# deezer/musicFPaugment

Measured on AMD Instinct MI355X. Metric: 8s/8kHz clips/sec (STFT+UNet+peak-pick), higher is better.
Workload: dtype bf16x3 (fp32 operands split into bf16 hi+lo, fp32 accumulate); 1 GPU; STFT(512/256,f64) -> UNet(1,1) eval forward (bf16x3 MFMA, formula weights) -> Audfprint peak-pick; 8 s / 8 kHz clips, 257x251 spectrograms; parallelism=clip-sharded x1, no data-path collective

## Files before the change

musicfpaugment_amd/csrc/unet.hip:

```cpp
#include "mfpa_common.h"
#include "mfpa_unet_args.h"

#include <cstdlib>
#include <type_traits>

namespace {

#ifdef MFPA_EXPERIMENTS
__device__ unsigned long long* mfpa_conv_stamps = nullptr;
#define MFPA_STAMP(slot)                                                                                                   \
  do {                                                                                                                     \
    if (mfpa_conv_stamps && threadIdx.x == 0)                                                                              \
      mfpa_conv_stamps[((size_t)blockIdx.y * gridDim.x + blockIdx.x) * 8 + (slot)] = __builtin_amdgcn_s_memrealtime();   \
  } while (0)
#else
#define MFPA_STAMP(slot) do { } while (0)
#endif

typedef float floatx16 __attribute__((ext_vector_type(16)));
typedef float f32x4 __attribute__((ext_vector_type(4)));
typedef __bf16 bf16x8 __attribute__((ext_vector_type(8)));
typedef __bf16 bf16x4 __attribute__((ext_vector_type(4)));
typedef __bf16 bf16x2 __attribute__((ext_vector_type(2)));
typedef float f32x2 __attribute__((ext_vector_type(2)));
// ... 591 lines not shown
    }
  }
  MFPA_STAMP(4);
}

typedef float floatx4 __attribute__((ext_vector_type(4)));

template <int CTRL>
__device__ __forceinline__ float dpp_row_add(float v) {
  return v + __int_as_float(__builtin_amdgcn_update_dpp(0, __float_as_int(v), CTRL, 0xf, 0xf, false));
}

template <int PH, int PW, bool ROWS, int WMW = 2, bool SIDE = false, bool PLAIN = false, bool IN16 = false, bool AFF16 = false>
__global__ __launch_bounds__(512, 1) void conv_wd16_kernel(ConvArgs a) {
  static_assert(!IN16 || PLAIN, "a bf16 source feeds the plain-bf16 products");
  constexpr int SPP = IN16 ? KC / 8 : KC / 4;
  constexpr int ESZ = IN16 ? 2 : 4;
  constexpr int THREADS = 512, WNW = 8 / WMW, BN = 32 * WNW, WPXW = 256 / WMW, TAPS = 9;
  static_assert((WMW == 2 || WMW == 4) && (!ROWS || WMW == 2), "wave grid");
  constexpr int HPW = PW + 2, HPH = PH + 2, HP = HPW * HPH, BM = PH * PW;
  static_assert(BM == 256 && (PW == 32 || PW == 16), "two waves of 128 pixels: eight 16-pixel tiles each");
  constexpr int A_F4 = (HP * SPP + THREADS - 1) / THREADS;
  constexpr int HPS = A_F4 * (THREADS / SPP);
  constexpr int PLANE = ((HPS * 16 + 255) / 256) * 256;
  constexpr int HLS = 4 * PLANE + 256;
  constexpr int STAGE = 2 * HLS;
  constexpr int PT = WPXW / 16;
  static_assert(A_F4 <= TAPS - 3, "one halo staging slot per tap, taps 2 .. 7");

  extern __shared__ __attribute__((aligned(16))) char smem[];
  const int tid = threadIdx.x, lane = tid & 63, wave = tid >> 6;
  const int wm = wave % WMW, wn = __builtin_amdgcn_readfirstlane(wave / WMW);
  const int p = lane & 15, g = lane >> 4;
  auto plane_off = [](int hl, int kg) { return hl * HLS + kg * PLANE + (kg >> 1) * 128; };

  constexpr bool PERSIST = (WMW == 4) || (!ROWS && !SIDE) || PLAIN;
  const int n0 = blockIdx.y * BN;
  const int Cin = a.C0 + a.C1;
  const int nchunks = Cin / KC;
  const int ntiles = a.tiles_x * a.tiles_y * a.B;

  const int aq = tid % SPP;
  constexpr int TBL = 2 * A_F4 * THREADS;
  unsigned* const aoffs0 = reinterpret_cast<unsigned*>(smem + 2 * STAGE);
#pragma unroll
  for (int it = 0; it < A_F4; ++it) {
    const int pix = tid / SPP + it * (THREADS / SPP);
    const int py = pix / HPW - 1, px = pix % HPW - 1;
    aoffs0[it * THREADS + tid] = (unsigned)((py * a.W + px) * a.C0 + (KC / SPP) * aq) * (unsigned)ESZ;
    aoffs0[(A_F4 + it) * THREADS + tid] = (unsigned)(((py - a.oy1) * a.W1 + (px - a.ox1)) * a.C1 + (KC / SPP) * aq) * (unsigned)ESZ;
  }
  typedef int i32x4_t __attribute__((ext_vector_type(4)));
  const unsigned clip0 = (unsigned)a.H * (unsigned)a.W * (unsigned)a.C0 * (unsigned)ESZ, clip1 = (unsigned)a.H1 * (unsigned)a.W1 * (unsigned)a.C1 * (unsigned)ESZ;
  struct Tile { int b, y0, x0p; unsigned ain; unsigned t0, t1; };
  auto make_tile = [&](int t) __attribute__((always_inline)) {
    Tile T;
    int bx = __builtin_amdgcn_readfirstlane(t);
// ... 101 lines not shown
        const float* scp = aff + c0 + 8 * aq;
        const float* shp = aff + a.C0 + c0 + 8 * aq;
        const f32x4 sc0 = *reinterpret_cast<const f32x4*>(scp), sc1 = *reinterpret_cast<const f32x4*>(scp + 4);
        const f32x4 sh0 = *reinterpret_cast<const f32x4*>(shp), sh1 = *reinterpret_cast<const f32x4*>(shp + 4);
#pragma unroll
        for (int k = 0; k < 8; ++k) {
          const float y = f[k] * (k < 4 ? sc0[k & 3] : sc1[k & 3]) + (k < 4 ? sh0[k & 3] : sh1[k & 3]);
          f[k] = y > 0.f ? y : 0.f;
        }
        if (a.drop_thresh) {
          const int gy = S.y0 + pix / HPW - 1, gx = S.x0p + pix % HPW - 1;
          const unsigned long long e0 = (((unsigned long long)S.b * a.H + gy) * a.W + gx) * a.C0 + c0 + 8 * aq;
#pragma unroll
          for (int k = 0; k < 8; ++k) f[k] = mfpa_keep(a.drop_seed, a.drop_thresh, e0 + k) ? f[k] * a.drop_scale : 0.f;
        }
#pragma unroll
        for (int k = 0; k < 4; ++k) {
          bf16x2 h2;
          h2[0] = (__bf16)f[2 * k];
          h2[1] = (__bf16)f[2 * k + 1];
          v[k] = __builtin_bit_cast(float, h2);
        }
      }
      *reinterpret_cast<f32x4*>(stage + plane_off(0, aq) + pix * 16) = v;
      if constexpr (SIDE && AFF16) {
        const int py = pix / HPW, px = pix % HPW;
        if (a.x0_bf16 != nullptr && c0 < a.C0 && inside && py >= 1 && py <= PH && px >= 1 && px <= PW && blockIdx.y == 0) {
          const size_t e = (size_t)S.b * a.H * a.W * a.C0 + ((aoffs0[it * THREADS + tid] + S.t0) >> 1) + c0;
          *reinterpret_cast<f32x4*>(a.x0_bf16 + e) = v;
        }
      }
      return;
    }
    if (a.in_scale0 != nullptr && c0 < a.C0 && inside) {
      const f32x4 sc = *reinterpret_cast<const f32x4*>(aff + c0 + 4 * aq);
      const f32x4 sh = *reinterpret_cast<const f32x4*>(aff + a.C0 + c0 + 4 * aq);
      v = v * sc + sh;
#pragma unroll
      for (int k = 0; k < 4; ++k) v[k] = v[k] > 0.f ? v[k] : 0.f;
      if (a.drop_thresh) {
        const int gy = S.y0 + pix / HPW - 1, gx = S.x0p + pix % HPW - 1;
        const unsigned long long e0 = (((unsigned long long)S.b * a.H + gy) * a.W + gx) * a.C0 + c0 + 4 * aq;
#pragma unroll
        for (int k = 0; k < 4; ++k) v[k] = mfpa_keep(a.drop_seed, a.drop_thresh, e0 + k) ? v[k] * a.drop_scale : 0.f;
      }
    }
    bf16x4 hi, lo;
#pragma unroll
    for (int k = 0; k < 4; ++k) {
      hi[k] = (__bf16)v[k];
      lo[k] = (__bf16)(v[k] - (float)hi[k]);
    }
    char* at = stage + plane_off(0, aq >> 1) + pix * 16 + 8 * (aq & 1);
    *reinterpret_cast<bf16x4*>(at) = hi;
    if constexpr (!PLAIN) *reinterpret_cast<bf16x4*>(at + HLS) = lo;
    if constexpr (SIDE) {
      const int py = pix / HPW, px = pix % HPW;
      const bool interior = inside && py >= 1 && py <= PH && px >= 1 && px <= PW && blockIdx.y == 0;
      if (a.x0_bf16 != nullptr && c0 < a.C0 && interior) {
        const size_t e = (size_t)S.b * a.H * a.W * a.C0 + ((aoffs0[it * THREADS + tid] + S.t0) >> 2) + c0;
        *reinterpret_cast<bf16x4*>(a.x0_bf16 + e) = hi;
      }
      if (a.x1_bf16 != nullptr && c0 >= a.C0 && interior) {
        const size_t e = (size_t)S.b * a.H1 * a.W1 * a.C1 + ((aoffs0[(A_F4 + it) * THREADS + tid] + S.t1) >> 2) + (c0 - a.C0);
        *reinterpret_cast<bf16x4*>(a.x1_bf16 + e) = hi;
      }
    }
  };

  bf16x8 wq[3][2][2];
  auto load_w = [&](int chunk, int tap, auto SLOT) __attribute__((always_inline)) {
    constexpr int slot = decltype(SLOT)::value;
    const char* wb = reinterpret_cast<const char*>(a.w) +
                     ((((size_t)tap * nchunks + chunk) * (size_t)(a.Cout / 16) + (size_t)(n0 / 16 + 2 * wn)) << 11) + lane * 16;
    wq[slot][0][0] = *reinterpret_cast<const bf16x8*>(wb);
    if constexpr (!PLAIN) wq[slot][0][1] = *reinterpret_cast<const bf16x8*>(wb + 1024);
    wq[slot][1][0] = *reinterpret_cast<const bf16x8*>(wb + 2048);
    if constexpr (!PLAIN) wq[slot][1][1] = *reinterpret_cast<const bf16x8*>(wb + 3072);
  };

  struct XFrags { bf16x8 h[4], l[4]; };
  XFrags fx0, fx1;
  const int xbase = (((wm * WPXW + p) / PW) * HPW + ((wm * WPXW + p) % PW)) * 16 + plane_off(0, g);
  auto tile_disp = [](int pt) { return (PW == 32) ? ((pt >> 1) * HPW + (pt & 1) * 16) * 16 : pt * HPW * 16; };
  auto read_x = [&](XFrags& f, const char* stage, int tap_off, int half) __attribute__((always_inline)) {
#pragma unroll
    for (int i = 0; i < 4; ++i) {
      const char* r = stage + xbase + tile_disp(4 * half + i) + tap_off;
      if constexpr (!PLAIN) f.l[i] = *reinterpret_cast<const bf16x8*>(r + HLS);
      f.h[i] = *reinterpret_cast<const bf16x8*>(r);
    }
  };
  floatx4 acc[2][PT];
#pragma unroll
  for (int ct = 0; ct < 2; ++ct)
#pragma unroll
    for (int pt = 0; pt < PT; ++pt) acc[ct][pt] = floatx4{0.f, 0.f, 0.f, 0.f};
  auto mfma_half = [&](const XFrags& f, const bf16x8 (&w)[2][2], int half) __attribute__((always_inline)) {
    if constexpr (!PLAIN) {
#pragma unroll
    for (int ct = 0; ct < 2; ++ct)
#pragma unroll
      for (int i = 0; i < 4; ++i) acc[ct][4 * half + i] = __builtin_amdgcn_mfma_f32_16x16x32_bf16(w[ct][1], f.h[i], acc[ct][4 * half + i], 0, 0, 0);
#pragma unroll
    for (int ct = 0; ct < 2; ++ct)
#pragma unroll
      for (int i = 0; i < 4; ++i) acc[ct][4 * half + i] = __builtin_amdgcn_mfma_f32_16x16x32_bf16(w[ct][0], f.l[i], acc[ct][4 * half + i], 0, 0, 0);
    }
#pragma unroll
    for (int ct = 0; ct < 2; ++ct)
#pragma unroll
      for (int i = 0; i < 4; ++i) acc[ct][4 * half + i] = __builtin_amdgcn_mfma_f32_16x16x32_bf16(w[ct][0], f.h[i], acc[ct][4 * half + i], 0, 0, 0);
  };
  using S0 = std::integral_constant<int, 0>;
  using S1 = std::integral_constant<int, 1>;
  constexpr int N_R = PLAIN ? 4 : 8, N_M = PLAIN ? 8 : 24;
  constexpr int N_W = PLAIN ? 2 : 4;
  auto tap_body = [&](auto TAP, int chunk) __attribute__((always_inline)) {
    constexpr int tap = decltype(TAP)::value;
    constexpr int ntap = (tap + 1) % TAPS;
    constexpr int tap_off = ((tap / 3) * HPW + (tap % 3)) * 16, ntap_off = ((ntap / 3) * HPW + (ntap % 3)) * 16;
    const int chunk_n = chunk + 1 < nchunks ? chunk + 1 : (PERSIST ? 0 : chunk);
    const char* cur = smem + (chunk & 1) * STAGE;
    const char* nxt = (tap == TAPS - 1) ? smem + ((chunk + 1) & 1) * STAGE : cur;
    read_x(fx1, cur, tap_off, 1);
    mfma_half(fx0, wq[tap % 3], 0);
    load_w((tap + 2 >= TAPS) ? chunk_n : chunk, (tap + 2) % TAPS, std::integral_constant<int, (tap + 2) % 3>{});
    pin_reads<N_M - 1, N_R>();
    constexpr int used_a = pin_read_slots(N_M - 1, N_R);
    __builtin_amdgcn_sched_group_barrier(0x008, 1, 0);
    __builtin_amdgcn_sched_group_barrier(0x020, N_W, 0);
    if constexpr (N_M - used_a - 1 > 0) __builtin_amdgcn_sched_group_barrier(0x008, N_M - used_a - 1, 0);
    __builtin_amdgcn_sched_barrier(0);
    if (tap == TAPS - 1) {
      __syncthreads();
      __builtin_amdgcn_sched_barrier(0);
    }
    if (tap == 0) load_a_pre(chunk_n);
    if (tap == TAPS - 1) preload_offsets(PERSIST ? (chunk + 2 < nchunks ? chunk + 2 : chunk + 1 < nchunks ? 0 : 1 < nchunks ? 1 : 0)
                                                 : (chunk + 2 < nchunks ? chunk + 2 : chunk + 1 < nchunks ? chunk + 1 : chunk));
    read_x(fx0, nxt, ntap_off, 0);
    mfma_half(fx1, wq[tap % 3], 1);
    if constexpr (tap >= 2 && tap - 2 < A_F4) {
      split_slot(std::integral_constant<int, tap - 2>{}, chunk_n, smem + ((chunk + 1) & 1) * STAGE);
#pragma unroll
      for (int i = 0; i < N_R; ++i) {
        __builtin_amdgcn_sched_group_barrier(0x008, 1, 0);
        __builtin_amdgcn_sched_group_barrier(0x100, 1, 0);
        __builtin_amdgcn_sched_group_barrier(0x002, 2, 0);
      }
#pragma unroll
      for (int i = 0; i < 2; ++i) {
        __builtin_amdgcn_sched_group_barrier(0x008, 2, 0);
        __builtin_amdgcn_sched_group_barrier(0x002, 4, 0);
        __builtin_amdgcn_sched_group_barrier(0x200, 1, 0);
      }
      if constexpr (N_M - N_R - 4 > 0) __builtin_amdgcn_sched_group_barrier(0x008, N_M - N_R - 4, 0);
    } else {
      pin_reads<N_M, N_R>();
      if constexpr (N_M - pin_read_slots(N_M, N_R) > 0) __builtin_amdgcn_sched_group_barrier(0x008, N_M - pin_read_slots(N_M, N_R), 0);
    }
    __builtin_amdgcn_sched_barrier(0);
  };

  auto tap_body4 = [&](auto TAP, auto PAR, int chunk) __attribute__((always_inline)) {
    constexpr int tap = decltype(TAP)::value, par = (decltype(PAR)::value + tap) & 1;
    constexpr int ntap = (tap + 1) % TAPS;
    constexpr int ntap_off = ((ntap / 3) * HPW + (ntap % 3)) * 16;
    const int chunk_n = chunk + 1 < nchunks ? chunk + 1 : 0;
    const char* cur = smem + (chunk & 1) * STAGE;
    const char* nxt = (tap == TAPS - 1) ? smem + ((chunk + 1) & 1) * STAGE : cur;
    stamp(tap);
    if (tap == TAPS - 1) {
      __syncthreads();
      __builtin_amdgcn_sched_barrier(0);
      stamp(9);
    }
    if (tap == 0) load_a_pre(chunk_n);
    if (tap == TAPS - 1) preload_offsets(chunk + 2 < nchunks ? chunk + 2 : chunk + 1 < nchunks ? 0 : 1 < nchunks ? 1 : 0);
    read_x(par ? fx0 : fx1, nxt, ntap_off, 0);
    if (!MFPA_EXP_FLAG(a.dbg, 8)) mfma_half(par ? fx1 : fx0, wq[tap % 3], 0);
    if (!MFPA_EXP_FLAG(a.dbg, 128)) load_w((tap + 2 >= TAPS) ? chunk_n : chunk, (tap + 2) % TAPS, std::integral_constant<int, (tap + 2) % 3>{});
    if constexpr (tap >= 2 && tap - 2 < A_F4) {
      if (!MFPA_EXP_FLAG(a.dbg, 256)) split_slot(std::integral_constant<int, tap - 2>{}, chunk_n, smem + ((chunk + 1) & 1) * STAGE);
#pragma unroll
      for (int i = 0; i < N_R; ++i) {
        __builtin_amdgcn_sched_group_barrier(0x008, 1, 0);
        __builtin_amdgcn_sched_group_barrier(0x100, 1, 0);
        __builtin_amdgcn_sched_group_barrier(0x002, 2, 0);
      }
#pragma unroll
// ... 33 lines not shown
    for (int dy = 0; dy < 3; ++dy) {
      const char* wb = reinterpret_cast<const char*>(a.w) +
                       ((((size_t)(dy * 3 + dx) * nchunks + chunk) * (size_t)(a.Cout / 16) + (size_t)(n0 / 16 + 2 * wn)) << 11) + lane * 16;
      wr[par][dy][0][0] = *reinterpret_cast<const bf16x8*>(wb);
      if constexpr (!PLAIN) wr[par][dy][0][1] = *reinterpret_cast<const bf16x8*>(wb + 1024);
      wr[par][dy][1][0] = *reinterpret_cast<const bf16x8*>(wb + 2048);
      if constexpr (!PLAIN) wr[par][dy][1][1] = *reinterpret_cast<const bf16x8*>(wb + 3072);
    }
  };
  constexpr int NU = (R + 2) * HV, NB = (PW == 32) ? 4 : 5;
  static_assert(NU % NB == 0, "static ring indices");
  auto load_wr1 = [&](int chunk, auto DX, auto PAR, auto DY) __attribute__((always_inline)) {
    constexpr int dx = decltype(DX)::value, par = decltype(PAR)::value, dy = decltype(DY)::value;
    const char* wb = reinterpret_cast<const char*>(a.w) +
                     ((((size_t)(dy * 3 + dx) * nchunks + chunk) * (size_t)(a.Cout / 16) + (size_t)(n0 / 16 + 2 * wn)) << 11) + lane * 16;
    wr[par][dy][0][0] = *reinterpret_cast<const bf16x8*>(wb);
    if constexpr (!PLAIN) wr[par][dy][0][1] = *reinterpret_cast<const bf16x8*>(wb + 1024);
    wr[par][dy][1][0] = *reinterpret_cast<const bf16x8*>(wb + 2048);
    if constexpr (!PLAIN) wr[par][dy][1][1] = *reinterpret_cast<const bf16x8*>(wb + 3072);
  };
  struct XUnit { bf16x8 h, l; };
  XUnit xu[NB];
  auto read_unit = [&](XUnit& f, const char* stage, int u, int dx) __attribute__((always_inline)) {
    const char* r = stage + xbase + ((u / HV) * HPW + (u % HV) * 16 + dx) * 16;
    if constexpr (!PLAIN) f.l = *reinterpret_cast<const bf16x8*>(r + HLS);
    f.h = *reinterpret_cast<const bf16x8*>(r);
  };
  auto mfma_unit = [&](auto U, const XUnit& f, auto PAR) __attribute__((always_inline)) {
    constexpr int h = decltype(U)::value / HV, hv = decltype(U)::value % HV, par = decltype(PAR)::value;
#pragma unroll
    for (int term = PLAIN ? 2 : 0; term < 3; ++term)
#pragma unroll
      for (int dy = 0; dy < 3; ++dy) {
        if (h - dy < 0 || h - dy >= R) continue;
#pragma unroll
        for (int ct = 0; ct < 2; ++ct) {
          floatx4& c = acc[ct][(h - dy) * HV + hv];
          c = __builtin_amdgcn_mfma_f32_16x16x32_bf16(wr[par][dy][ct][term == 0 ? 1 : 0], term == 1 ? f.l : f.h, c, 0, 0, 0);
        }
      }
  };
  auto unit_mfmas = [](int u) { const int h = u / HV; int n = 0; for (int dy = 0; dy < 3; ++dy) n += (h - dy >= 0 && h - dy < R) ? 1 : 0; return n * (PLAIN ? 2 : 6); };
  constexpr int BARU = NU - NB + 1;
  constexpr int SA = NU / 2, SB = BARU - AHALF;
  static_assert(SA + AHALF < NU && SB >= 0, "staging schedule");
  auto unit_step = [&](auto U, auto DX, auto PAR, int chunk) __attribute__((always_inline)) {
    constexpr int u = decltype(U)::value, dx = decltype(DX)::value, par = decltype(PAR)::value;
// ... 375 lines not shown
    tap_body(std::integral_constant<int, 5>{}, chunk);
    tap_body(std::integral_constant<int, 6>{}, chunk);
    tap_body(std::integral_constant<int, 7>{}, chunk);
    tap_body(std::integral_constant<int, 8>{}, chunk);
  }
  epilogue();
  }
}

constexpr int CONV_WD16_ROWS = 512;

template <int PH, int PW, int WMW = 2>
int launch_wd16(ConvArgs& a, hipStream_t s) {
  a.tiles_x = (a.W + PW - 1) / PW;
  a.tiles_y = (a.H + PH - 1) / PH;
  static const int dbg_env = MFPA_EXP_ENV("MFPA_CONV_DBG", 0);
  a.dbg = dbg_env;
  static const int stagger_env = MFPA_EXP_ENV("MFPA_CONV_STAGGER", 0);
  a.dbg_stagger = stagger_env;
  if ((long long)a.tiles_x * a.tiles_y * a.B > 0x7fffffffLL) return MFPA_EINVAL;
  constexpr int HP = (PW + 2) * (PH + 2);
  constexpr int A_F4 = (HP * (KC / 4) + 511) / 512;
  constexpr int HPS = A_F4 * 64;
  constexpr int PLANE = ((HPS * 16 + 255) / 256) * 256;
  const size_t lds = 2 * (size_t)(2 * (4 * PLANE + 256)) + (size_t)2 * A_F4 * 512 * sizeof(unsigned) +
                     (a.in_scale0 ? (size_t)2 * a.C0 * sizeof(float) : 0) +
                     (a.w1x1 ? (size_t)2 * 256 * sizeof(float) : 0) +
                     (size_t)(2 * 32 * (8 / WMW) + 64) * sizeof(float);
  dim3 grid((unsigned)((long long)a.tiles_x * a.tiles_y * a.B), (unsigned)(a.Cout / (32 * (8 / WMW))));
#ifdef MFPA_EXPERIMENTS
  a.dbg_lds_stamps = (int)lds;
  const_cast<size_t&>(lds) += 4096;
#endif
  const int cin = a.C0 + a.C1;
  const bool side = a.x0_bf16 || a.x1_bf16 || a.y_bf16 || a.stats_part;
  const bool rows = WMW == 2 && cin % 64 == 0 && cin >= CONV_WD16_ROWS;
  if (WMW == 4 || a.plain || (!side && !rows)) {
    const int cus = mfpa_current_device_cus();
    const unsigned per = (unsigned)((cus > 0 ? cus : 256) / (int)grid.y);
    if (per >= 1 && grid.x > per) grid.x = per;
  }
  if (a.in16) {
    if (!a.plain || a.x1_bf16 || cin % 64) return MFPA_EINVAL;
    const bool fwd16 = a.in_scale0 != nullptr || a.x0_bf16 != nullptr || (a.y == nullptr && a.bz == nullptr);
    if constexpr (WMW == 4) {
      if (fwd16) hipLaunchKernelGGL((conv_wd16_kernel<PH, PW, false, 4, true, true, true, true>), grid, dim3(512), lds, s, a);
      else if (side) hipLaunchKernelGGL((conv_wd16_kernel<PH, PW, false, 4, true, true, true>), grid, dim3(512), lds, s, a);
      else hipLaunchKernelGGL((conv_wd16_kernel<PH, PW, false, 4, false, true, true>), grid, dim3(512), lds, s, a);
// ... 656 lines not shown
```

musicfpaugment_amd/csrc/unet_up.hip:

```cpp
#include "mfpa_common.h"
#include "mfpa_unet_args.h"

#include <type_traits>

namespace mfpa_unet {
namespace {

typedef float f32x4 __attribute__((ext_vector_type(4)));
typedef float floatx4 __attribute__((ext_vector_type(4)));
typedef __bf16 bf16x8 __attribute__((ext_vector_type(8)));
typedef float f32x2 __attribute__((ext_vector_type(2)));
typedef __bf16 bf16x2 __attribute__((ext_vector_type(2)));

constexpr int KC = 32;
constexpr int PH = 8, PW = 32, HPW = PW + 2, HPH = PH + 2, HP = HPW * HPH;
constexpr int HALF = HPW / 2;
constexpr int LPH = PH / 2 + 2, LPW = PW / 2 + 2, LP = LPH * LPW;
constexpr int THREADS = 512, LTHREADS = 256;
constexpr int SPP = KC / 4;
constexpr int PPI = LTHREADS / SPP;
constexpr int A_F4 = (HP + PPI - 1) / PPI;
constexpr int L_F4 = (LP + PPI - 1) / PPI;
constexpr int HPS = A_F4 * PPI;
constexpr int PLANE = ((HPS * 16 + 255) / 256) * 256;
constexpr int HLS = 4 * PLANE + 256;
constexpr int STAGE = 2 * HLS;
constexpr int PT = 8;
constexpr int EPI_FLOATS = 64 + 16 * 64;
constexpr int OUTBUF = PH * PW * 64 * 4;

__device__ __forceinline__ constexpr int plane_off(int hl, int kg) { return hl * HLS + kg * PLANE + (kg >> 1) * 128; }

template <int SLOTS, int LEFT, int I = 0>
__device__ __forceinline__ void pin_reads() {
  if constexpr (I < SLOTS && LEFT > 0) {
    constexpr int k = (LEFT + (SLOTS - I) - 1) / (SLOTS - I);
    __builtin_amdgcn_sched_group_barrier(0x008, 1, 0);
    __builtin_amdgcn_sched_group_barrier(0x100, k, 0);
    pin_reads<SLOTS, LEFT - k, I + 1>();
  }
}
constexpr int pin_read_slots(int slots, int left) {
  int used = 0;
  for (int i = 0; i < slots && left > 0; ++i) {
    left -= (left + (slots - i) - 1) / (slots - i);
    ++used;
  }
  return used;
}

__device__ __forceinline__ int tile_of(int b, int i, int G, int ngrp) {
  if (ngrp == 1 && (G & 7) == 0) return i * G + (b & 7) * (G >> 3) + (b >> 3);
  return i * G + b;
}
// ... 94 lines not shown
    }
    const unsigned clip0 = (unsigned)a.H * (unsigned)a.W * (unsigned)a.Cs * 4u, clip1 = (unsigned)a.Hl * (unsigned)a.Wl * (unsigned)a.Cl * 4u;
    f32x4 areg[2][A_F4] = {};
    struct Src { __amdgpu_buffer_rsrc_t rs; unsigned toff; bool from0, interior; int ainsh; };
    auto make_src = [&](const Tile& T, int chunk) __attribute__((always_inline)) {
      Src S;
      S.from0 = chunk < nsk;
      const char* pb = reinterpret_cast<const char*>(S.from0 ? a.skip : a.low) + (size_t)T.b * (S.from0 ? clip0 : clip1);
      S.rs = __builtin_amdgcn_make_buffer_rsrc(const_cast<char*>(pb), 0, (int)(S.from0 ? clip0 : clip1), 0x00020000);
      S.toff = S.from0 ? T.t0 + (unsigned)(chunk * KC) * 4u : T.t1 + (unsigned)((chunk - nsk) * KC) * 4u;
      S.interior = S.from0 ? T.int0 : T.int1;
      S.ainsh = S.from0 ? 0 : 16;
      return S;
    };
    auto issue_slot = [&](const Src& S, unsigned ain, unsigned tab, auto INTERIOR, auto SET, auto IT) __attribute__((always_inline)) {
      constexpr int it = decltype(IT)::value, set = decltype(SET)::value;
      if constexpr (decltype(INTERIOR)::value) {
        areg[set][it] = __builtin_bit_cast(f32x4, __builtin_amdgcn_raw_buffer_load_b128(S.rs, (int)tab, (int)S.toff, 0));
      } else {
        const bool inside = (ain >> (S.ainsh + it)) & 1u;
        areg[set][it] = __builtin_bit_cast(f32x4, __builtin_amdgcn_raw_buffer_load_b128(S.rs, (int)(inside ? tab + S.toff : 0xfffffff0u), 0, 0));
      }
    };
    char* const wbase = smem + plane_off(0, aq >> 1) + pl * 16 + 8 * (aq & 1);
    char* const wbase32 = smem + plane_off(aq >> 2, aq & 3) + pl * 16;
    auto split_slot = [&](auto SET, auto IT, int stage_off) __attribute__((always_inline)) {
      constexpr int it = decltype(IT)::value, set = decltype(SET)::value;
      const f32x4 v = areg[set][it];
      if constexpr (PREC == 0) {
        *reinterpret_cast<f32x4*>(wbase32 + stage_off + it * PPI * 16) = v;
        return;
      }
      unsigned hi[2], lo[2];
#pragma unroll
      for (int h = 0; h < 2; ++h) {
        const f32x2 x = {v[2 * h], v[2 * h + 1]};
        hi[h] = __builtin_bit_cast(unsigned, __builtin_convertvector(x, bf16x2));
        const f32x2 r = {x[0] - __uint_as_float(hi[h] << 16), x[1] - __uint_as_float(hi[h] & 0xffff0000u)};
        lo[h] = __builtin_bit_cast(unsigned, __builtin_convertvector(r, bf16x2));
      }
      char* at = wbase + stage_off + it * PPI * 16;
      *reinterpret_cast<uint2*>(at) = uint2{hi[0], hi[1]};
      *reinterpret_cast<uint2*>(at + HLS) = uint2{lo[0], lo[1]};
    };
    static_assert(A_F4 == 11 && L_F4 == 4, "eleven / four staging slots per loader thread");
#define MFPA_UP_EACH4(M) M(0) M(1) M(2) M(3)
#define MFPA_UP_EACH7(M) M(4) M(5) M(6) M(7) M(8) M(9) M(10)
    auto issue_all = [&](const Src& S, unsigned ain, auto SET) __attribute__((always_inline)) {
      if (S.from0) {
        if (S.interior) {
#define MFPA_UP_ISSUE(I) issue_slot(S, ain, off0[I], std::true_type{}, SET, std::integral_constant<int, I>{});
          MFPA_UP_EACH4(MFPA_UP_ISSUE) MFPA_UP_EACH7(MFPA_UP_ISSUE)
#undef MFPA_UP_ISSUE
        } else {
#define MFPA_UP_ISSUE(I) issue_slot(S, ain, off0[I], std::false_type{}, SET, std::integral_constant<int, I>{});
          MFPA_UP_EACH4(MFPA_UP_ISSUE) MFPA_UP_EACH7(MFPA_UP_ISSUE)
#undef MFPA_UP_ISSUE
        }
      } else {
        if (S.interior) {
#define MFPA_UP_ISSUE(I) issue_slot(S, ain, off1[I], std::true_type{}, SET, std::integral_constant<int, I>{});
          MFPA_UP_EACH4(MFPA_UP_ISSUE)
#undef MFPA_UP_ISSUE
        } else {
// ... 52 lines not shown
  const int wlane = lane * 16;
  auto load_w_at = [&](__amdgpu_buffer_rsrc_t rs, unsigned blk, auto SLOT) __attribute__((always_inline)) {
    constexpr int slot = decltype(SLOT)::value;
    const int so = (int)__builtin_amdgcn_readfirstlane((int)(blk << 11));
    wq[slot][0][0] = __builtin_bit_cast(frag_t, __builtin_amdgcn_raw_buffer_load_b128(rs, wlane, so, 0));
    wq[slot][0][1] = __builtin_bit_cast(frag_t, __builtin_amdgcn_raw_buffer_load_b128(rs, wlane + 1024, so, 0));
    wq[slot][1][0] = __builtin_bit_cast(frag_t, __builtin_amdgcn_raw_buffer_load_b128(rs, wlane + 2048, so, 0));
    wq[slot][1][1] = __builtin_bit_cast(frag_t, __builtin_amdgcn_raw_buffer_load_b128(rs, wlane + 3072, so, 0));
  };
#ifdef MFPA_UP_WHOT
#define MFPA_UP_WBLK(x) (wcol)
#else
#define MFPA_UP_WBLK(x) (x)
#endif
  auto load_w_skip = [&](int chunk, int tap, auto SLOT) __attribute__((always_inline)) {
    load_w_at(rs_skip, MFPA_UP_WBLK(((unsigned)tap * (unsigned)nsk + (unsigned)chunk) * wrow + wcol), SLOT);
  };
  auto load_w_up = [&](int chunk, int pair, int px, auto SLOT) __attribute__((always_inline)) {
    const unsigned t16 = (unsigned)((wm * 2 + px) * 4 + pair);
    load_w_at(rs_up, MFPA_UP_WBLK((t16 * (unsigned)nup + (unsigned)chunk) * wrow + wcol), SLOT);
  };
  struct XFrags { frag_t h[4], l[4]; };
  XFrags fx0, fx1;
  const int pl0 = PREC == 1 ? plane_off(0, g) : plane_off(g >> 1, 2 * (g & 1));
  constexpr int SECOND = PREC == 1 ? HLS : PLANE;
  const int xb_skip = (wm * HPW + p) * 16 + pl0;
  const int xb_up = (wm * LPW + p) * 16 + pl0;
  auto read_at = [&](XFrags& f, const char* base, auto STRIDE) __attribute__((always_inline)) {
    constexpr int stride = decltype(STRIDE)::value;
#pragma unroll
    for (int j = 0; j < 4; ++j) {
      const char* r = base + j * stride;
      f.l[j] = *reinterpret_cast<const frag_t*>(r + SECOND);
      f.h[j] = *reinterpret_cast<const frag_t*>(r);
    }
  };
  auto read_skip = [&](XFrags& f, const char* stage, auto TAP, auto PX) __attribute__((always_inline)) {
    constexpr int tap = decltype(TAP)::value, s = decltype(PX)::value + tap % 3;
    read_at(f, stage + xb_skip + ((tap / 3) * HPW + (s & 1) * HALF + (s >> 1)) * 16, std::integral_constant<int, 2 * HPW * 16>{});
  };
  auto read_up = [&](XFrags& f, const char* stage, auto PAIR, auto PX) __attribute__((always_inline)) {
    constexpr int pair = decltype(PAIR)::value;
    read_at(f, stage + xb_up + ((pair >> 1) * LPW + (pair & 1) + decltype(PX)::value) * 16, std::integral_constant<int, LPW * 16>{});
  };
  floatx4 acc[2][PT];
#pragma unroll
  for (int ct = 0; ct < 2; ++ct)
#pragma unroll
    for (int pt = 0; pt < PT; ++pt) acc[ct][pt] = floatx4{0.f, 0.f, 0.f, 0.f};
  floatx4 initv[2];
  auto mfma_half = [&](const XFrags& f, const frag_t (&w)[2][2], auto HALFI, auto FIRST) __attribute__((always_inline)) {
    constexpr int half = decltype(HALFI)::value;
    if constexpr (PREC == 0) {
#pragma unroll
      for (int s8 = 0; s8 < 8; ++s8)
#pragma unroll
        for (int ct = 0; ct < 2; ++ct)
#pragma unroll
          for (int i = 0; i < 4; ++i) {
            const float wv = (s8 < 4 ? w[ct][0] : w[ct][1])[s8 & 3], xv = (s8 < 4 ? f.h[i] : f.l[i])[s8 & 3];
            acc[ct][4 * half + i] = __builtin_amdgcn_mfma_f32_16x16x4f32(wv, xv, (decltype(FIRST)::value && s8 == 0) ? initv[ct] : acc[ct][4 * half + i], 0, 0, 0);
          }
      return;
    } else {
#pragma unroll
    for (int ct = 0; ct < 2; ++ct)
// ... 242 lines not shown
```

musicfpaugment_amd/csrc/unet_ws.hip:

```cpp
#include "mfpa_common.h"
#include "mfpa_unet_args.h"

#include <type_traits>

namespace mfpa_unet {
#if defined(MFPA_EXPERIMENTS) || defined(MFPA_WS_STAMPS)
__device__ unsigned long long* ws_stamps = nullptr;
#endif
namespace {

typedef float f32x4 __attribute__((ext_vector_type(4)));
typedef float floatx4 __attribute__((ext_vector_type(4)));
typedef __bf16 bf16x8 __attribute__((ext_vector_type(8)));
typedef __bf16 bf16x4 __attribute__((ext_vector_type(4)));
typedef float f32x2 __attribute__((ext_vector_type(2)));
typedef __bf16 bf16x2 __attribute__((ext_vector_type(2)));

#ifndef MFPA_WS_COMPUTE_PRIO
#define MFPA_WS_COMPUTE_PRIO 0
#endif
#ifndef MFPA_WS_LOADER_PRIO
#define MFPA_WS_LOADER_PRIO 0
#endif
#ifndef MFPA_WS_EPI_PRIO
// ... 8 lines not shown
#ifndef MFPA_WS_XCD_TILES
#define MFPA_WS_XCD_TILES 1
#endif

#ifdef MFPA_SKIP_BITS
#define WS_FLAG(bit) (((MFPA_SKIP_BITS) & (bit)) != 0)
#else
#define WS_FLAG(bit) false
#endif
#if defined(MFPA_EXPERIMENTS) && !defined(MFPA_WS_STAMPS)
#define MFPA_WS_STAMPS 1
#endif
#ifdef MFPA_WS_STAMPS
constexpr int WS_MAX_STAMPS = 128;
#endif

constexpr int KC = 32;
constexpr int PH = 8, PW = 32, HPW = PW + 2, HPH = PH + 2, HP = HPW * HPH;
constexpr int THREADS = 512, LTHREADS = 256;
constexpr int SPP = KC / 4;
constexpr int PPI = LTHREADS / SPP;
constexpr int A_F4 = (HP + PPI - 1) / PPI;
constexpr int HPS = A_F4 * PPI;
constexpr int PLANE = ((HPS * 16 + 255) / 256) * 256;
constexpr int HLS = 4 * PLANE + 256;
constexpr int STAGE = 2 * HLS;
constexpr int TAPS = 9, PT = 8;
constexpr int OUTBUF = PH * PW * 64 * 4;
constexpr int C1W = PW + 4, C1PROWS = 6;
constexpr int C1LDS = (4 * C1PROWS * C1W + 128) * 4;

__device__ __forceinline__ constexpr int plane_off(int hl, int kg) { return hl * HLS + kg * PLANE + (kg >> 1) * 128; }

template <int SLOTS, int LEFT, int I = 0>
__device__ __forceinline__ void pin_reads() {
  if constexpr (I < SLOTS && LEFT > 0) {
    constexpr int k = (LEFT + (SLOTS - I) - 1) / (SLOTS - I);
    __builtin_amdgcn_sched_group_barrier(0x008, 1, 0);
    __builtin_amdgcn_sched_group_barrier(0x100, k, 0);
    pin_reads<SLOTS, LEFT - k, I + 1>();
  }
}
constexpr int pin_read_slots(int slots, int left) {
  int used = 0;
  for (int i = 0; i < slots && left > 0; ++i) {
    left -= (left + (slots - i) - 1) / (slots - i);
    ++used;
  }
  return used;
}

__device__ __forceinline__ int tile_of(int b, int i, int G) {
#if MFPA_WS_XCD_TILES
  if ((G & 7) == 0) return i * G + (b & 7) * (G >> 3) + (b >> 3);
#endif
// ... 210 lines not shown
        S.from0 = c0 < a.C0;
        const char* pb = reinterpret_cast<const char*>(S.from0 ? a.x0 : a.x1) + (size_t)T.b * (S.from0 ? clip0 : clip1);
        S.rs = __builtin_amdgcn_make_buffer_rsrc(const_cast<char*>(pb), 0, (int)(S.from0 ? clip0 : clip1), 0x00020000);
        S.toff = S.from0 ? T.t0 + (unsigned)c0 * 4u : T.t1 + (unsigned)(c0 - a.C0) * 4u;
        S.ainsh = S.from0 ? 0 : 16;
        return S;
      };
      auto issue_slot = [&](const Src& S, unsigned ain, auto SET, auto IT) __attribute__((always_inline)) {
        constexpr int it = decltype(IT)::value, set = decltype(SET)::value;
        unsigned o0 = off0[it], o1 = off1[it];
        asm("" : "+v"(o0), "+v"(o1));
        const bool inside = (ain >> (S.ainsh + it)) & 1u;
        const unsigned off = inside ? (S.from0 ? o0 : o1) + S.toff : 0xfffffff0u;
        if (WS_FLAG(1) || WS_FLAG(32)) return;
        areg[set][it] = __builtin_bit_cast(f32x4, __builtin_amdgcn_raw_buffer_load_b128(S.rs, (int)off, 0, 0));
        if (MFPA_WS_PACE) __builtin_amdgcn_s_sleep(MFPA_WS_PACE);
      };
      auto issue_slot_interior = [&](const Src& S, auto FROM0, auto SET, auto IT) __attribute__((always_inline)) {
        constexpr int it = decltype(IT)::value, set = decltype(SET)::value;
        if (WS_FLAG(1) || WS_FLAG(32)) return;
        areg[set][it] = __builtin_bit_cast(f32x4, __builtin_amdgcn_raw_buffer_load_b128(S.rs, (int)(decltype(FROM0)::value ? off0[it] : off1[it]), (int)S.toff, 0));
        if (MFPA_WS_PACE) __builtin_amdgcn_s_sleep(MFPA_WS_PACE);
      };
      char* const wbase = smem + plane_off(0, aq >> 1) + (lt / SPP) * 16 + 8 * (aq & 1);
      char* const wbase_split = smem + plane_off(aq >> 2, aq & 3) + (lt / SPP) * 16;
      auto copy_slot = [&](auto SET, auto IT, int stage_off) __attribute__((always_inline)) {
        constexpr int it = decltype(IT)::value, set = decltype(SET)::value;
        if (WS_FLAG(1)) return;
        *reinterpret_cast<f32x4*>(wbase_split + stage_off + it * PPI * 16) = areg[set][it];
      };
      auto split_slot = [&](auto SET, auto IT, int stage_off) __attribute__((always_inline)) {
        constexpr int it = decltype(IT)::value, set = decltype(SET)::value;
        if (WS_FLAG(1)) return;
        const f32x4 v = areg[set][it];
        unsigned hi[2], lo[2];
#pragma unroll
        for (int h = 0; h < 2; ++h) {
          const f32x2 x = {v[2 * h], v[2 * h + 1]};
          hi[h] = __builtin_bit_cast(unsigned, __builtin_convertvector(x, bf16x2));
          const f32x2 r = {x[0] - __uint_as_float(hi[h] << 16), x[1] - __uint_as_float(hi[h] & 0xffff0000u)};
          lo[h] = __builtin_bit_cast(unsigned, __builtin_convertvector(r, bf16x2));
        }
        char* at = wbase + stage_off + it * PPI * 16;
        if (WS_FLAG(64)) {
          if (hi[0] + hi[1] + lo[0] + lo[1] == 0x12345678u) *reinterpret_cast<uint2*>(at) = uint2{hi[0], hi[1]};
          return;
        }
        *reinterpret_cast<uint2*>(at) = uint2{hi[0], hi[1]};
        *reinterpret_cast<uint2*>(at + HLS) = uint2{lo[0], lo[1]};
      };
      static_assert(A_F4 == 11, "eleven staging slots per loader thread");
      auto issue_all = [&](const Src& S, unsigned ain, bool interior, auto SET) __attribute__((always_inline)) {
        if (interior) {
          if (S.from0) {
#define MFPA_WS_ISSUE(I) issue_slot_interior(S, std::true_type{}, SET, std::integral_constant<int, I>{});
            MFPA_WS_ISSUE(0) MFPA_WS_ISSUE(1) MFPA_WS_ISSUE(2) MFPA_WS_ISSUE(3) MFPA_WS_ISSUE(4) MFPA_WS_ISSUE(5)
            MFPA_WS_ISSUE(6) MFPA_WS_ISSUE(7) MFPA_WS_ISSUE(8) MFPA_WS_ISSUE(9) MFPA_WS_ISSUE(10)
#undef MFPA_WS_ISSUE
          } else {
#define MFPA_WS_ISSUE(I) issue_slot_interior(S, std::false_type{}, SET, std::integral_constant<int, I>{});
            MFPA_WS_ISSUE(0) MFPA_WS_ISSUE(1) MFPA_WS_ISSUE(2) MFPA_WS_ISSUE(3) MFPA_WS_ISSUE(4) MFPA_WS_ISSUE(5)
            MFPA_WS_ISSUE(6) MFPA_WS_ISSUE(7) MFPA_WS_ISSUE(8) MFPA_WS_ISSUE(9) MFPA_WS_ISSUE(10)
#undef MFPA_WS_ISSUE
          }
          return;
        }
// ... 172 lines not shown
      };
      auto produce = [&](int c, int stage_off) __attribute__((always_inline)) {
#pragma unroll
        for (int cth = 0; cth < 2; ++cth) {
          const int ct = 2 * c + cth;
          const f32x4 sc = *reinterpret_cast<const f32x4*>(c1c + 16 * ct + 4 * g);
          const f32x4 sh = *reinterpret_cast<const f32x4*>(c1c + 64 + 16 * ct + 4 * g);
          const s16x4 ah = c ? (cth ? Ahi[3] : Ahi[2]) : (cth ? Ahi[1] : Ahi[0]);
          const s16x4 al = c ? (cth ? Alo[3] : Alo[2]) : (cth ? Alo[1] : Alo[0]);
#pragma unroll
          for (int tt = 0; tt < 6; ++tt) {
            if (tt >= npt) continue;
            floatx4 d = {0.f, 0.f, 0.f, 0.f};
            d = __builtin_amdgcn_mfma_f32_16x16x16bf16_1k(al, Bh[tt], d, 0, 0, 0);
            d = __builtin_amdgcn_mfma_f32_16x16x16bf16_1k(ah, Bl[tt], d, 0, 0, 0);
            d = __builtin_amdgcn_mfma_f32_16x16x16bf16_1k(ah, Bh[tt], d, 0, 0, 0);
            const bool in = (inside >> tt) & 1u;
            float v[4];
#pragma unroll
            for (int j = 0; j < 4; ++j) v[j] = in ? fmaxf(fmaf(d[j], sc[j], sh[j]), 0.f) : 0.f;
            unsigned h0, l0, h1, l1;
            split2(v[0], v[1], h0, l0);
            split2(v[2], v[3], h1, l1);
            char* at = smem + stage_off + plane_off(0, cth * 2 + (g >> 1)) + ((pt0 + tt) * 16 + p) * 16 + 8 * (g & 1);
            *reinterpret_cast<uint2*>(at) = uint2{h0, h1};
            *reinterpret_cast<uint2*>(at + HLS) = uint2{l0, l1};
          }
        }
      };
      const int total = owned * 2;
      int par = 0;
      request_patch(tile_of((int)blockIdx.x, 0, G));
      for (int k = -1; k < total; ++k) {
        stamp(20);
        if (k + 1 < total) {
          const int i = (k + 1) >> 1, c = (k + 1) & 1;
          if (c == 0) {
            commit_patch();
            build_b(tile_of((int)blockIdx.x, i, G));
            if (i + 1 < owned) request_patch(tile_of((int)blockIdx.x, i + 1, G));
          }
          produce(c, par * STAGE);
        }
        stamp(22);
        if (has_duty && k >= 3 && (k - 1) % 2 == 0) duty(tile_of((int)blockIdx.x, (k - 1) / 2 - 1, G));
        stamp(24);
        __syncthreads();
// ... 8 lines not shown
    dump_stamps();
    return;
  }

#if MFPA_WS_COMPUTE_PRIO
  __builtin_amdgcn_s_setprio(MFPA_WS_COMPUTE_PRIO);
#endif
  const int wm = wave & 1, wn = wave >> 1;
  const int p = lane & 15, g = lane >> 4;

  bool primed = false;
  bf16x8 wq[3][2][2];
  auto load_w = [&](int chunk, int tap, auto SLOT) __attribute__((always_inline)) {
    constexpr int slot = decltype(SLOT)::value;
    if (WS_FLAG(16) && primed) return;
    const char* wb = reinterpret_cast<const char*>(a.w) + ((((size_t)tap * nchunks + chunk) * (size_t)(a.Cout / 16) + (size_t)(n0 / 16 + 2 * wn)) << 11) + lane * 16;
    wq[slot][0][0] = *reinterpret_cast<const bf16x8*>(wb);
    wq[slot][0][1] = *reinterpret_cast<const bf16x8*>(wb + 1024);
    wq[slot][1][0] = *reinterpret_cast<const bf16x8*>(wb + 2048);
    wq[slot][1][1] = *reinterpret_cast<const bf16x8*>(wb + 3072);
  };
  struct XFrags { bf16x8 h[4], l[4]; };
  XFrags fx0, fx1;
  const int xbase = ((4 * wm) * HPW + p) * 16 + plane_off(0, g);
  auto tile_disp = [](int pt) { return ((pt >> 1) * HPW + (pt & 1) * 16) * 16; };
  auto read_x = [&](XFrags& f, const char* stage, int tap_off, int half) __attribute__((always_inline)) {
    if (WS_FLAG(8)) return;
#pragma unroll
    for (int i = 0; i < 4; ++i) {
      const char* r = stage + xbase + tile_disp(4 * half + i) + tap_off;
      f.l[i] = *reinterpret_cast<const bf16x8*>(r + HLS);
      f.h[i] = *reinterpret_cast<const bf16x8*>(r);
    }
  };
  floatx4 acc[2][PT];
#pragma unroll
  for (int ct = 0; ct < 2; ++ct)
#pragma unroll
    for (int pt = 0; pt < PT; ++pt) acc[ct][pt] = floatx4{0.f, 0.f, 0.f, 0.f};
  floatx4 initv[2];
  auto mfma_half = [&](const XFrags& f, const bf16x8 (&w)[2][2], int half, auto FIRST) __attribute__((always_inline)) {
#pragma unroll
    for (int ct = 0; ct < 2; ++ct)
#pragma unroll
      for (int i = 0; i < 4; ++i)
        acc[ct][4 * half + i] = __builtin_amdgcn_mfma_f32_16x16x32_bf16(w[ct][1], f.h[i], decltype(FIRST)::value ? initv[ct] : acc[ct][4 * half + i], 0, 0, 0);
#pragma unroll
    for (int ct = 0; ct < 2; ++ct)
#pragma unroll
      for (int i = 0; i < 4; ++i) acc[ct][4 * half + i] = __builtin_amdgcn_mfma_f32_16x16x32_bf16(w[ct][0], f.l[i], acc[ct][4 * half + i], 0, 0, 0);
#pragma unroll
    for (int ct = 0; ct < 2; ++ct)
#pragma unroll
      for (int i = 0; i < 4; ++i) acc[ct][4 * half + i] = __builtin_amdgcn_mfma_f32_16x16x32_bf16(w[ct][0], f.h[i], acc[ct][4 * half + i], 0, 0, 0);
  };
  constexpr int N_R = 8, N_M = 24, N_W = 4;
  int kpar = 0;
#if MFPA_WS_SYNC
  unsigned gck = 0, rdy_early = 0;
  const unsigned total_c = (unsigned)(owned * nchunks);
#endif
  auto tap_body = [&](auto TAP, int chunk, auto FIRST) __attribute__((always_inline)) {
    constexpr int tap = decltype(TAP)::value;
    constexpr int ntap = (tap + 1) % TAPS;
    constexpr int tap_off = ((tap / 3) * HPW + (tap % 3)) * 16, ntap_off = ((ntap / 3) * HPW + (ntap % 3)) * 16;
    const int chunk_n = chunk + 1 < nchunks ? chunk + 1 : 0;
    const char* cur = smem + kpar * STAGE;
    const char* nxt = (tap == TAPS - 1) ? smem + (kpar ^ 1) * STAGE : cur;
    stamp(tap);
    read_x(fx1, cur, tap_off, 1);
    mfma_half(fx0, wq[tap % 3], 0, FIRST);
    load_w((tap + 2 >= TAPS) ? chunk_n : chunk, (tap + 2) % TAPS, std::integral_constant<int, (tap + 2) % 3>{});
    pin_reads<N_M - 1, N_R>();
    constexpr int used_a = pin_read_slots(N_M - 1, N_R);
    __builtin_amdgcn_sched_group_barrier(0x008, 1, 0);
    __builtin_amdgcn_sched_group_barrier(0x020, N_W, 0);
    if constexpr (N_M - used_a - 1 > 0) __builtin_amdgcn_sched_group_barrier(0x008, N_M - used_a - 1, 0);
    __builtin_amdgcn_sched_barrier(0);
#if MFPA_WS_SYNC
    if (tap == TAPS - 2) rdy_early = peek(READY);
#endif
    if (tap == TAPS - 1) {
      stamp(9);
#if MFPA_WS_SYNC
      publish(FREED, gck + 1u);
      if (gck + 1u < total_c && (unsigned)__builtin_amdgcn_readfirstlane((int)rdy_early) < gck + 2u) wait_for(READY, gck + 2u);
      ++gck;
#else
// ... 200 lines not shown
```

Baseline: 5231 clips/s.

## Interleave channel-group pairs per pixel in conv LDS staging with padded planes

Replaces the per-kernel LDS staging layout, one 16-byte plane per channel group, with a shared layout that packs two channel groups into a 32-byte pixel record across two planes. Plane and half-stage sizes are padded to fixed residues mod 128 bytes to change bank mapping. The aim is to reduce LDS bank conflicts on fragment reads and staging stores across the down, up and warp-specialised conv kernels. Because the layout must agree between every store site and every read site, any missed or mismatched offset would corrupt results. The new padding also changes the LDS footprint.

```diff
diff --git a/musicfpaugment_amd/csrc/mfpa_conv_lds.h b/musicfpaugment_amd/csrc/mfpa_conv_lds.h
--- /dev/null
+++ b/musicfpaugment_amd/csrc/mfpa_conv_lds.h
@@ -0,0 +1,38 @@
+#ifndef MFPA_CONV_LDS_H
+#define MFPA_CONV_LDS_H
+
+#if defined(__HIPCC__) || defined(__CUDACC__)
+#define MFPA_LDS_FN __host__ __device__ __forceinline__ constexpr
+#else
+#define MFPA_LDS_FN inline constexpr
+#endif
+
+namespace mfpa_conv_lds {
+
+constexpr int PIX = 32;
+
+template <int HPS>
+struct Stage {
+  static constexpr int PLANE = ((HPS * PIX + 63) / 128) * 128 + 64;
+  static constexpr int HLS = 2 * PLANE + 32;
+  static constexpr int STAGE = 2 * HLS;
+  static_assert(PLANE >= HPS * PIX && PLANE % 128 == 64 && HLS % 128 == 32, "the residues the stores rely on");
+
+  static MFPA_LDS_FN int plane_off(int hl, int kg) { return hl * HLS + (kg >> 1) * PLANE + (kg & 1) * 16; }
+  static MFPA_LDS_FN int pix_off(int pixels) { return pixels * PIX; }
+
+  static MFPA_LDS_FN int split_store_off(int pixel, int aq) { return plane_off(0, aq >> 1) + pixel * PIX + 8 * (aq & 1); }
+  static MFPA_LDS_FN int copy_store_off(int pixel, int aq) { return plane_off(aq >> 2, aq & 3) + pixel * PIX; }
+  static MFPA_LDS_FN int bf16_store_off(int pixel, int kg) { return plane_off(0, kg) + pixel * PIX; }
+  static MFPA_LDS_FN int f32_store_off(int pixel, int aq) { return plane_off(aq >> 2, ((aq & 1) << 1) | ((aq >> 1) & 1)) + pixel * PIX; }
+
+  static MFPA_LDS_FN int frag_off(int hl, int g) { return plane_off(hl, g); }
+  static MFPA_LDS_FN int f32_frag_off(int g, int second) { return f32_store_off(0, 2 * g + second); }
+  static constexpr int F32_SECOND = PLANE;
+};
+
+MFPA_LDS_FN int out_tile_off(int m, int q) { return m * 256 + ((q ^ (m & 15)) << 4); }
+
+}
+
+#endif
diff --git a/musicfpaugment_amd/csrc/unet.hip b/musicfpaugment_amd/csrc/unet.hip
--- a/musicfpaugment_amd/csrc/unet.hip
+++ b/musicfpaugment_amd/csrc/unet.hip
@@ -1,4 +1,5 @@
 #include "mfpa_common.h"
+#include "mfpa_conv_lds.h"
 #include "mfpa_unet_args.h"
 
 #include <cstdlib>
@@ -637,9 +638,8 @@
   static_assert(BM == 256 && (PW == 32 || PW == 16), "two waves of 128 pixels: eight 16-pixel tiles each");
   constexpr int A_F4 = (HP * SPP + THREADS - 1) / THREADS;
   constexpr int HPS = A_F4 * (THREADS / SPP);
-  constexpr int PLANE = ((HPS * 16 + 255) / 256) * 256;
-  constexpr int HLS = 4 * PLANE + 256;
-  constexpr int STAGE = 2 * HLS;
+  using LDS = mfpa_conv_lds::Stage<HPS>;
+  constexpr int HLS = LDS::HLS, STAGE = LDS::STAGE;
   constexpr int PT = WPXW / 16;
   static_assert(A_F4 <= TAPS - 3, "one halo staging slot per tap, taps 2 .. 7");
 
@@ -647,7 +647,6 @@
   const int tid = threadIdx.x, lane = tid & 63, wave = tid >> 6;
   const int wm = wave % WMW, wn = __builtin_amdgcn_readfirstlane(wave / WMW);
   const int p = lane & 15, g = lane >> 4;
-  auto plane_off = [](int hl, int kg) { return hl * HLS + kg * PLANE + (kg >> 1) * 128; };
 
   constexpr bool PERSIST = (WMW == 4) || (!ROWS && !SIDE) || PLAIN;
   const int n0 = blockIdx.y * BN;
@@ -795,7 +794,7 @@
           v[k] = __builtin_bit_cast(float, h2);
         }
       }
-      *reinterpret_cast<f32x4*>(stage + plane_off(0, aq) + pix * 16) = v;
+      *reinterpret_cast<f32x4*>(stage + LDS::bf16_store_off(pix, aq)) = v;
       if constexpr (SIDE && AFF16) {
         const int py = pix / HPW, px = pix % HPW;
         if (a.x0_bf16 != nullptr && c0 < a.C0 && inside && py >= 1 && py <= PH && px >= 1 && px <= PW && blockIdx.y == 0) {
@@ -824,7 +823,7 @@
       hi[k] = (__bf16)v[k];
       lo[k] = (__bf16)(v[k] - (float)hi[k]);
     }
-    char* at = stage + plane_off(0, aq >> 1) + pix * 16 + 8 * (aq & 1);
+    char* at = stage + LDS::split_store_off(pix, aq);
     *reinterpret_cast<bf16x4*>(at) = hi;
     if constexpr (!PLAIN) *reinterpret_cast<bf16x4*>(at + HLS) = lo;
     if constexpr (SIDE) {
@@ -854,8 +853,8 @@
 
   struct XFrags { bf16x8 h[4], l[4]; };
   XFrags fx0, fx1;
-  const int xbase = (((wm * WPXW + p) / PW) * HPW + ((wm * WPXW + p) % PW)) * 16 + plane_off(0, g);
-  auto tile_disp = [](int pt) { return (PW == 32) ? ((pt >> 1) * HPW + (pt & 1) * 16) * 16 : pt * HPW * 16; };
+  const int xbase = LDS::pix_off(((wm * WPXW + p) / PW) * HPW + ((wm * WPXW + p) % PW)) + LDS::frag_off(0, g);
+  auto tile_disp = [](int pt) { return LDS::pix_off((PW == 32) ? (pt >> 1) * HPW + (pt & 1) * 16 : pt * HPW); };
   auto read_x = [&](XFrags& f, const char* stage, int tap_off, int half) __attribute__((always_inline)) {
 #pragma unroll
     for (int i = 0; i < 4; ++i) {
@@ -892,7 +891,7 @@
   auto tap_body = [&](auto TAP, int chunk) __attribute__((always_inline)) {
     constexpr int tap = decltype(TAP)::value;
     constexpr int ntap = (tap + 1) % TAPS;
-    constexpr int tap_off = ((tap / 3) * HPW + (tap % 3)) * 16, ntap_off = ((ntap / 3) * HPW + (ntap % 3)) * 16;
+    constexpr int tap_off = LDS::pix_off((tap / 3) * HPW + (tap % 3)), ntap_off = LDS::pix_off((ntap / 3) * HPW + (ntap % 3));
     const int chunk_n = chunk + 1 < nchunks ? chunk + 1 : (PERSIST ? 0 : chunk);
     const char* cur = smem + (chunk & 1) * STAGE;
     const char* nxt = (tap == TAPS - 1) ? smem + ((chunk + 1) & 1) * STAGE : cur;
@@ -939,7 +938,7 @@
   auto tap_body4 = [&](auto TAP, auto PAR, int chunk) __attribute__((always_inline)) {
     constexpr int tap = decltype(TAP)::value, par = (decltype(PAR)::value + tap) & 1;
     constexpr int ntap = (tap + 1) % TAPS;
-    constexpr int ntap_off = ((ntap / 3) * HPW + (ntap % 3)) * 16;
+    constexpr int ntap_off = LDS::pix_off((ntap / 3) * HPW + (ntap % 3));
     const int chunk_n = chunk + 1 < nchunks ? chunk + 1 : 0;
     const char* cur = smem + (chunk & 1) * STAGE;
     const char* nxt = (tap == TAPS - 1) ? smem + ((chunk + 1) & 1) * STAGE : cur;
@@ -1019,7 +1018,7 @@
   struct XUnit { bf16x8 h, l; };
   XUnit xu[NB];
   auto read_unit = [&](XUnit& f, const char* stage, int u, int dx) __attribute__((always_inline)) {
-    const char* r = stage + xbase + ((u / HV) * HPW + (u % HV) * 16 + dx) * 16;
+    const char* r = stage + xbase + LDS::pix_off((u / HV) * HPW + (u % HV) * 16 + dx);
     if constexpr (!PLAIN) f.l = *reinterpret_cast<const bf16x8*>(r + HLS);
     f.h = *reinterpret_cast<const bf16x8*>(r);
   };
@@ -1441,8 +1440,7 @@
   constexpr int HP = (PW + 2) * (PH + 2);
   constexpr int A_F4 = (HP * (KC / 4) + 511) / 512;
   constexpr int HPS = A_F4 * 64;
-  constexpr int PLANE = ((HPS * 16 + 255) / 256) * 256;
-  const size_t lds = 2 * (size_t)(2 * (4 * PLANE + 256)) + (size_t)2 * A_F4 * 512 * sizeof(unsigned) +
+  const size_t lds = 2 * (size_t)mfpa_conv_lds::Stage<HPS>::STAGE + (size_t)2 * A_F4 * 512 * sizeof(unsigned) +
                      (a.in_scale0 ? (size_t)2 * a.C0 * sizeof(float) : 0) +
                      (a.w1x1 ? (size_t)2 * 256 * sizeof(float) : 0) +
                      (size_t)(2 * 32 * (8 / WMW) + 64) * sizeof(float);
diff --git a/musicfpaugment_amd/csrc/unet_up.hip b/musicfpaugment_amd/csrc/unet_up.hip
--- a/musicfpaugment_amd/csrc/unet_up.hip
+++ b/musicfpaugment_amd/csrc/unet_up.hip
@@ -1,4 +1,5 @@
 #include "mfpa_common.h"
+#include "mfpa_conv_lds.h"
 #include "mfpa_unet_args.h"
 
 #include <type_traits>
@@ -22,14 +23,11 @@
 constexpr int A_F4 = (HP + PPI - 1) / PPI;
 constexpr int L_F4 = (LP + PPI - 1) / PPI;
 constexpr int HPS = A_F4 * PPI;
-constexpr int PLANE = ((HPS * 16 + 255) / 256) * 256;
-constexpr int HLS = 4 * PLANE + 256;
-constexpr int STAGE = 2 * HLS;
+using LDS = mfpa_conv_lds::Stage<HPS>;
+constexpr int HLS = LDS::HLS, STAGE = LDS::STAGE;
 constexpr int PT = 8;
 constexpr int EPI_FLOATS = 64 + 16 * 64;
 constexpr int OUTBUF = PH * PW * 64 * 4;
-
-__device__ __forceinline__ constexpr int plane_off(int hl, int kg) { return hl * HLS + kg * PLANE + (kg >> 1) * 128; }
 
 template <int SLOTS, int LEFT, int I = 0>
 __device__ __forceinline__ void pin_reads() {
@@ -170,13 +168,13 @@
         areg[set][it] = __builtin_bit_cast(f32x4, __builtin_amdgcn_raw_buffer_load_b128(S.rs, (int)(inside ? tab + S.toff : 0xfffffff0u), 0, 0));
       }
     };
-    char* const wbase = smem + plane_off(0, aq >> 1) + pl * 16 + 8 * (aq & 1);
-    char* const wbase32 = smem + plane_off(aq >> 2, aq & 3) + pl * 16;
+    char* const wbase = smem + LDS::split_store_off(pl, aq);
+    char* const wbase32 = smem + LDS::f32_store_off(pl, aq);
     auto split_slot = [&](auto SET, auto IT, int stage_off) __attribute__((always_inline)) {
       constexpr int it = decltype(IT)::value, set = decltype(SET)::value;
       const f32x4 v = areg[set][it];
       if constexpr (PREC == 0) {
-        *reinterpret_cast<f32x4*>(wbase32 + stage_off + it * PPI * 16) = v;
+        *reinterpret_cast<f32x4*>(wbase32 + stage_off + LDS::pix_off(it * PPI)) = v;
         return;
       }
       unsigned hi[2], lo[2];
@@ -187,7 +185,7 @@
         const f32x2 r = {x[0] - __uint_as_float(hi[h] << 16), x[1] - __uint_as_float(hi[h] & 0xffff0000u)};
         lo[h] = __builtin_bit_cast(unsigned, __builtin_convertvector(r, bf16x2));
       }
-      char* at = wbase + stage_off + it * PPI * 16;
+      char* at = wbase + stage_off + LDS::pix_off(it * PPI);
       *reinterpret_cast<uint2*>(at) = uint2{hi[0], hi[1]};
       *reinterpret_cast<uint2*>(at + HLS) = uint2{lo[0], lo[1]};
     };
@@ -286,10 +284,10 @@
   };
   struct XFrags { frag_t h[4], l[4]; };
   XFrags fx0, fx1;
-  const int pl0 = PREC == 1 ? plane_off(0, g) : plane_off(g >> 1, 2 * (g & 1));
-  constexpr int SECOND = PREC == 1 ? HLS : PLANE;
-  const int xb_skip = (wm * HPW + p) * 16 + pl0;
-  const int xb_up = (wm * LPW + p) * 16 + pl0;
+  const int pl0 = PREC == 1 ? LDS::frag_off(0, g) : LDS::f32_frag_off(g, 0);
+  constexpr int SECOND = PREC == 1 ? HLS : LDS::F32_SECOND;
+  const int xb_skip = LDS::pix_off(wm * HPW + p) + pl0;
+  const int xb_up = LDS::pix_off(wm * LPW + p) + pl0;
   auto read_at = [&](XFrags& f, const char* base, auto STRIDE) __attribute__((always_inline)) {
     constexpr int stride = decltype(STRIDE)::value;
 #pragma unroll
@@ -301,11 +299,11 @@
   };
   auto read_skip = [&](XFrags& f, const char* stage, auto TAP, auto PX) __attribute__((always_inline)) {
     constexpr int tap = decltype(TAP)::value, s = decltype(PX)::value + tap % 3;
-    read_at(f, stage + xb_skip + ((tap / 3) * HPW + (s & 1) * HALF + (s >> 1)) * 16, std::integral_constant<int, 2 * HPW * 16>{});
+    read_at(f, stage + xb_skip + LDS::pix_off((tap / 3) * HPW + (s & 1) * HALF + (s >> 1)), std::integral_constant<int, LDS::pix_off(2 * HPW)>{});
   };
   auto read_up = [&](XFrags& f, const char* stage, auto PAIR, auto PX) __attribute__((always_inline)) {
     constexpr int pair = decltype(PAIR)::value;
-    read_at(f, stage + xb_up + ((pair >> 1) * LPW + (pair & 1) + decltype(PX)::value) * 16, std::integral_constant<int, LPW * 16>{});
+    read_at(f, stage + xb_up + LDS::pix_off((pair >> 1) * LPW + (pair & 1) + decltype(PX)::value), std::integral_constant<int, LDS::pix_off(LPW)>{});
   };
   floatx4 acc[2][PT];
 #pragma unroll
diff --git a/musicfpaugment_amd/csrc/unet_ws.hip b/musicfpaugment_amd/csrc/unet_ws.hip
--- a/musicfpaugment_amd/csrc/unet_ws.hip
+++ b/musicfpaugment_amd/csrc/unet_ws.hip
@@ -1,4 +1,5 @@
 #include "mfpa_common.h"
+#include "mfpa_conv_lds.h"
 #include "mfpa_unet_args.h"
 
 #include <type_traits>
@@ -54,15 +55,12 @@
 constexpr int PPI = LTHREADS / SPP;
 constexpr int A_F4 = (HP + PPI - 1) / PPI;
 constexpr int HPS = A_F4 * PPI;
-constexpr int PLANE = ((HPS * 16 + 255) / 256) * 256;
-constexpr int HLS = 4 * PLANE + 256;
-constexpr int STAGE = 2 * HLS;
+using LDS = mfpa_conv_lds::Stage<HPS>;
+constexpr int HLS = LDS::HLS, STAGE = LDS::STAGE;
 constexpr int TAPS = 9, PT = 8;
 constexpr int OUTBUF = PH * PW * 64 * 4;
 constexpr int C1W = PW + 4, C1PROWS = 6;
 constexpr int C1LDS = (4 * C1PROWS * C1W + 128) * 4;
-
-__device__ __forceinline__ constexpr int plane_off(int hl, int kg) { return hl * HLS + kg * PLANE + (kg >> 1) * 128; }
 
 template <int SLOTS, int LEFT, int I = 0>
 __device__ __forceinline__ void pin_reads() {
@@ -319,12 +317,12 @@
         areg[set][it] = __builtin_bit_cast(f32x4, __builtin_amdgcn_raw_buffer_load_b128(S.rs, (int)(decltype(FROM0)::value ? off0[it] : off1[it]), (int)S.toff, 0));
         if (MFPA_WS_PACE) __builtin_amdgcn_s_sleep(MFPA_WS_PACE);
       };
-      char* const wbase = smem + plane_off(0, aq >> 1) + (lt / SPP) * 16 + 8 * (aq & 1);
-      char* const wbase_split = smem + plane_off(aq >> 2, aq & 3) + (lt / SPP) * 16;
+      char* const wbase = smem + LDS::split_store_off(lt / SPP, aq);
+      char* const wbase_split = smem + LDS::copy_store_off(lt / SPP, aq);
       auto copy_slot = [&](auto SET, auto IT, int stage_off) __attribute__((always_inline)) {
         constexpr int it = decltype(IT)::value, set = decltype(SET)::value;
         if (WS_FLAG(1)) return;
-        *reinterpret_cast<f32x4*>(wbase_split + stage_off + it * PPI * 16) = areg[set][it];
+        *reinterpret_cast<f32x4*>(wbase_split + stage_off + LDS::pix_off(it * PPI)) = areg[set][it];
       };
       auto split_slot = [&](auto SET, auto IT, int stage_off) __attribute__((always_inline)) {
         constexpr int it = decltype(IT)::value, set = decltype(SET)::value;
@@ -338,7 +336,7 @@
           const f32x2 r = {x[0] - __uint_as_float(hi[h] << 16), x[1] - __uint_as_float(hi[h] & 0xffff0000u)};
           lo[h] = __builtin_bit_cast(unsigned, __builtin_convertvector(r, bf16x2));
         }
-        char* at = wbase + stage_off + it * PPI * 16;
+        char* at = wbase + stage_off + LDS::pix_off(it * PPI);
         if (WS_FLAG(64)) {
           if (hi[0] + hi[1] + lo[0] + lo[1] == 0x12345678u) *reinterpret_cast<uint2*>(at) = uint2{hi[0], hi[1]};
           return;
@@ -557,7 +555,7 @@
             unsigned h0, l0, h1, l1;
             split2(v[0], v[1], h0, l0);
             split2(v[2], v[3], h1, l1);
-            char* at = smem + stage_off + plane_off(0, cth * 2 + (g >> 1)) + ((pt0 + tt) * 16 + p) * 16 + 8 * (g & 1);
+            char* at = smem + stage_off + LDS::split_store_off((pt0 + tt) * 16 + p, 2 * (cth * 2 + (g >> 1)) + (g & 1));
             *reinterpret_cast<uint2*>(at) = uint2{h0, h1};
             *reinterpret_cast<uint2*>(at + HLS) = uint2{l0, l1};
           }
@@ -612,8 +610,8 @@
   };
   struct XFrags { bf16x8 h[4], l[4]; };
   XFrags fx0, fx1;
-  const int xbase = ((4 * wm) * HPW + p) * 16 + plane_off(0, g);
-  auto tile_disp = [](int pt) { return ((pt >> 1) * HPW + (pt & 1) * 16) * 16; };
+  const int xbase = LDS::pix_off((4 * wm) * HPW + p) + LDS::frag_off(0, g);
+  auto tile_disp = [](int pt) { return LDS::pix_off((pt >> 1) * HPW + (pt & 1) * 16); };
   auto read_x = [&](XFrags& f, const char* stage, int tap_off, int half) __attribute__((always_inline)) {
     if (WS_FLAG(8)) return;
 #pragma unroll
@@ -653,7 +651,7 @@
   auto tap_body = [&](auto TAP, int chunk, auto FIRST) __attribute__((always_inline)) {
     constexpr int tap = decltype(TAP)::value;
     constexpr int ntap = (tap + 1) % TAPS;
-    constexpr int tap_off = ((tap / 3) * HPW + (tap % 3)) * 16, ntap_off = ((ntap / 3) * HPW + (ntap % 3)) * 16;
+    constexpr int tap_off = LDS::pix_off((tap / 3) * HPW + (tap % 3)), ntap_off = LDS::pix_off((ntap / 3) * HPW + (ntap % 3));
     const int chunk_n = chunk + 1 < nchunks ? chunk + 1 : 0;
     const char* cur = smem + kpar * STAGE;
     const char* nxt = (tap == TAPS - 1) ? smem + (kpar ^ 1) * STAGE : cur;
```

Result: no change. 5266 clips/s (median of 6 runs) (+0.7%).
